# ffreyer/MonteCarlo.jl

Hardware: AMD Instinct MI355X
Metric: DQMC sweeps/sec, 16x16 Hubbard beta=8 dtau=0.1; achieved % fp64 MFMA roofline (higher is better)
Workload: dtype f64

## Files before the change

### montecarlo.jl_amd/csrc/engine.cpp

```cpp
#include <hip/hip_runtime.h>

#include <algorithm>
#include <cmath>
#include <cstdio>
#include <cstdlib>
#include <cstring>
#include <string>
#include <vector>

#include "../../include/dqmc_hip.h"
#include "kernels.h"
#include <rccl/rccl.h>

using namespace dqmc;

struct dqmc_comm {
    ncclComm_t comm = nullptr;
    int nranks = 1, rank = 0, device = 0;
};

static thread_local std::string g_create_error;

struct UTStack;

// ... 374 lines not shown
    if (const char *e = getenv("DQMC_QRB_SITES")) k.qrb_sites = atoi(e) & 7;
    if (const char *e = getenv("DQMC_QR_TAIL")) k.qr_tail = atoi(e) != 0;
    k.qr_sc1 = getenv("DQMC_QR_SC1") != nullptr;
    k.qr_nocoop = getenv("DQMC_QR_NOCOOP") != nullptr;
    if (const char *e = getenv("DQMC_QR_FORCE_TIMEOUT"))
        k.qr_force_timeout = strncmp(e, "step:", 5) == 0 ? 2 + atoi(e + 5) : (strncmp(e, "extra:", 6) == 0 ? 1000 + atoi(e + 6) : 1);
    k.qr_nopanel = getenv("DQMC_QR_NOPANEL") != nullptr;
    k.trsm_simple = getenv("DQMC_TRSM_SIMPLE") != nullptr;
    k.sweep_split = getenv("DQMC_SWEEP_SPLIT") != nullptr;
    k.flush_ncp2 = getenv("DQMC_FLUSH_NCP2") != nullptr;
    k.no_slab = getenv("DQMC_NO_SLAB") != nullptr;
    k.no_kron = getenv("DQMC_NO_KRON") != nullptr;
    k.no_wrap_flush = getenv("DQMC_NO_WRAP_FLUSH") != nullptr;
    k.wrap_two_launch = getenv("DQMC_WRAP_TWO_LAUNCH") != nullptr;
    k.tdm_general = getenv("DQMC_TDM_GENERAL") != nullptr;
}

static int alloc_qr_workspace(dqmc_handle *h)
{
    CHK(dalloc(h, &h->qr_ws.errflag, (size_t)1));
    h->qr_ws.tail = h->sw.qr_tail;
    h->qr_ws.force_sc1 = h->sw.qr_sc1;
    h->qr_ws.no_coop = h->sw.qr_nocoop;
    h->qr_ws.no_panel = h->sw.qr_nopanel;
    h->qr_ws.force_timeout = h->sw.qr_force_timeout;
    if (h->n > 256) return 0;
    hipDeviceProp_t prop;
    HIPCHK(hipGetDeviceProperties(&prop, h->p.device_id));
    const size_t slots = (size_t)((h->units + 7) / 8) * 8 * QR_COOP_SLOTS_PER_UNIT;
    CHK(dalloc(h, &h->qr_ws.mailbox, slots * QR_COOP_SLOT));
// ... 89 lines not shown
    if (udt_is_fused(h, 0) && Tout && Tout != A) return udt_fused(h, A, Uout, Dout, Tout, apply, h->qs[0]);
    CHK(udt_factor(h, A, Dout, Tout, apply, h->qs[0]));
    return udt_formq(h, Uout, h->qs[0], h->qs[0].winv, h->qs[0].ts);
}
static int rdivp_set(dqmc_handle *h, const double *A, const double *T, double *Out, const QrSet &q, double *winv, double *ts)
{
    Timed t(h, DQMC_K_TRSM);
    HIPCHK(launch_trsm_right_upper(h->n, h->units, A, h->nn, T, h->nn, q.pivot, nullptr, 0, Out, h->nn, winv, h->sw, h->cur, ts));
    return 0;
}
static int rdivp(dqmc_handle *h, double *A, const double *T)
{
    return rdivp_set(h, A, T, A, h->qs[0], h->qs[0].winv, h->qs[0].ts);
}

static int calculate_greens_src(dqmc_handle *h, double *out, Udt L, Udt R, double *a2_copy = nullptr)
{
    const int n = h->n;
    QrSet &qa = h->qs[0], &qb = h->qs[0];
    GemmArgs g = gemm_base(h, U_(h, L.t), 0, U_(h, R.t), 1, out);
    g.colscale = vs_arr(R.d, n);
    g.rowscale = vs_arr(L.d, n);
    CHK(run_gemm(h, g));
    if (udt_is_fused(h, 1)) {
        if (L.u == h->Tl) return fail(h, DQMC_ERR_STATE, "calculate_greens: Ul aliases Tl");
        CHK(udt_fused(h, out, h->Tl, h->Dr, qa.W, 0, qa, L.u));
        CHK(rdivp_set(h, R.u, qa.W, h->Ur, qa, qa.winv, qa.ts));
    } else {
        CHK(udt_factor(h, out, h->Dr, nullptr, 0, qa));
        CHK(rdivp_set(h, R.u, out, h->Ur, qa, qa.winv, qa.ts));
        CHK(udt_formq(h, h->Tr, qa, qa.winv, qa.ts));
// ... 4 lines not shown
    CHK(run_gemm(h, g));
    if (a2_copy) CHK(copy_mat(h, a2_copy, h->Tr));
    const double *tlul = h->Tr;
    if (udt_is_fused(h, 2)) {
        CHK(udt_fused(h, h->Tr, h->Ul, h->Dr, qb.W, 0, qb, h->Tl));
        CHK(rdivp_set(h, h->Ur, qb.W, h->Ur, qb, qb.winv, qb.ts));
        tlul = h->Ul;
    } else {
        CHK(udt_factor(h, h->Tr, h->Dr, nullptr, 0, qb));
        CHK(rdivp_set(h, h->Ur, h->Tr, h->Ur, qb, qb.winv, qb.ts));
        CHK(udt_formq(h, h->Ul, qb, qb.winv, qb.ts));
        CHK(run_gemm(h, gemm_base(h, U_(h, h->Tl), 0, U_(h, h->Ul), 0, h->Tr)));
    }
    g = gemm_base(h, U_(h, h->Ur), 0, U_(h, tlul), 1, out);
    g.kscale = vs_inv(h->Dr, n);
    CHK(run_gemm(h, g));
    return 0;
}
static int calculate_greens(dqmc_handle *h, double *out, double *a2_copy = nullptr)
{
    return calculate_greens_src(h, out, Udt{h->Ul, h->Dl, h->Tl}, Udt{h->Ur, h->Dr, h->Tr}, a2_copy);
}

enum { CB_LEFT_B = 0, CB_LEFT_BINV = 1, CB_LEFT_BDAG = 2, CB_RIGHT_B = 3, CB_RIGHT_BINV = 4, CB_RIGHT_ET = 5,
       CB_LEFT_ETINV = 6 };
static int cb_mult(dqmc_handle *h, int which, int slice, const double *X, double *O, const double *qscale)
{
    CbArgs a{};
    a.n = h->n; a.nb = h->nb; a.kmax = h->cb.kmax;
    a.side = (which == CB_RIGHT_B || which == CB_RIGHT_BINV || which == CB_RIGHT_ET) ? 1 : 0;
// ... 271 lines not shown
}

static int reset_slot(dqmc_handle *h, int slot)
{
    const int sp = h->K + 1;
    CHK(set_identity(h, uslot(h, sp)));
    CHK(set_ones(h, dslot(h, sp)));
    CHK(set_identity(h, tslot(h, sp)));
    slot_swap_spare(h, slot);
    return 0;
}
static int prop_check(dqmc_handle *h)
{
    Timed t(h, DQMC_K_MISC);
    HIPCHK(launch_prop_check(h->n, h->nb, h->W, h->greens_temp, h->greens, h->nn, h->stats, h->pc_scratch, h->cur));
    return 0;
}

static int init_stack(dqmc_handle *h)
{
    CHK(set_identity(h, h->Ul)); CHK(set_identity(h, h->Ur));
    CHK(set_identity(h, h->Tl)); CHK(set_identity(h, h->Tr));
    CHK(set_ones(h, h->Dl)); CHK(set_ones(h, h->Dr));
    h->current_slice = 0;
    h->direction = 0;
    return 0;
}
static int build_stack(dqmc_handle *h)
{
    CHK(reset_slot(h, 0));
// ... 15 lines not shown
                discard_pending_flush(h);
                CHK(calculate_greens_src(h, h->greens, slot_ref(h, 0), R));
            } else if (1 < h->current_slice && h->current_slice <= M) {
                const int idx = (h->current_slice - 1) / s;
                const Udt R = slot_ref(h, idx);
                const bool wt = h->p.check_propagation_error != 0, wt_slab = wt && oop_wrap(h);
                CHK(add_slice_sequence_left(h, idx, wt_slab));
                const Udt L = slot_ref(h, idx);
                if (wt && !wt_slab) {
                    CHK(materialize_pending_flush(h));
                    CHK(copy_mat(h, h->greens_temp, h->greens));
                    CHK(wrap_greens(h, &h->greens_temp, h->current_slice - 1, 1));
                }
                if (wt_slab) {
                    std::swap(h->greens, h->greens_alt);
                    CHK(calculate_greens_src(h, h->greens, L, R));
                    CHK(prop_check(h));
                    return 0;
                }
                discard_pending_flush(h);
                CHK(calculate_greens_src(h, h->greens, L, R));
                if (h->p.check_propagation_error) CHK(prop_check(h));
            } else {
                CHK(add_slice_sequence_left(h, h->K));
                h->direction = -1;
                h->current_slice = M + 1;
                CHK(propagate(h));
            }
        } else {
            CHK(wrap_greens(h, &h->greens, h->current_slice, 1));
            h->current_slice += 1;
        }
    } else {
        if ((h->current_slice - 1) % s == 0) {
            h->current_slice -= 1;
            if (h->current_slice == M) {
                const Udt L = slot_ref(h, h->K);
                CHK(reset_slot(h, h->K));
                discard_pending_flush(h);
                CHK(calculate_greens_src(h, h->greens, L, slot_ref(h, h->K)));
                CHK(wrap_greens(h, &h->greens, h->current_slice + 1, -1));
            } else if (0 < h->current_slice && h->current_slice < M) {
                const int idx = h->current_slice / s + 1;
                const Udt L = slot_ref(h, idx - 1);
                CHK(add_slice_sequence_right(h, idx));
                const Udt R = slot_ref(h, idx - 1);
                if (h->p.check_propagation_error) {
                    CHK(materialize_pending_flush(h));
                    std::swap(h->greens_temp, h->greens);
                }
                discard_pending_flush(h);
                CHK(calculate_greens_src(h, h->greens, L, R));
                if (h->p.check_propagation_error) CHK(prop_check(h));
                CHK(wrap_greens(h, &h->greens, h->current_slice + 1, -1));
            } else {
                CHK(add_slice_sequence_right(h, 1));
                h->direction = 1;
                h->current_slice = 0;
                CHK(propagate(h));
            }
        } else {
            CHK(wrap_greens(h, &h->greens, h->current_slice, -1));
            h->current_slice -= 1;
        }
    }
    return 0;
}

// ... 1239 lines not shown
```

### montecarlo.jl_amd/csrc/gemm_f64.hip

```cpp
#include "kernels.h"
#include <hip/hip_ext.h>
#include <cstdlib>

namespace dqmc {

typedef double d4 __attribute__((ext_vector_type(4)));

constexpr int BM = 64, BN = 64, BK = 16;
constexpr int LS = 80;

template <bool KCONTIG, bool FULL>
__device__ __forceinline__ void tile_load(const double *__restrict__ p, int ld, int c0, int cdim,
                                          int k0, int kdim, int tid, double r[4])
{
    if (FULL) {
        const double *q = KCONTIG ? p + (long)ld * (c0 + (tid >> 2)) + k0 + ((tid & 3) << 2)
                                  : p + (long)ld * (k0 + (tid >> 4)) + c0 + ((tid & 15) << 2);
        r[0] = q[0]; r[1] = q[1]; r[2] = q[2]; r[3] = q[3];
        return;
    }
    if (!KCONTIG) {
        const int kk = k0 + (tid >> 4), cc = c0 + ((tid & 15) << 2);
        const double *q = p + (long)ld * kk + cc;
        if (kk < kdim && cc + 3 < cdim) {
// ... 18 lines not shown
__device__ __forceinline__ void tile_store(double (*Xs)[LS], int tid, const double r[4])
{
    if (!KCONTIG) {
        const int k = tid >> 4;
        double *d = &Xs[k][(((tid & 15) << 2) + ((k >> 2) << 2)) & 63];
        d[0] = r[0]; d[1] = r[1]; d[2] = r[2]; d[3] = r[3];
    } else {
        const int c = tid >> 2, k = (tid & 3) << 2;
#pragma unroll
        for (int i = 0; i < 4; ++i) Xs[k + i][(c + k) & 63] = r[i];
    }
}

#define GEMM_LDS_BARRIER() asm volatile("s_waitcnt lgkmcnt(0)\n\ts_barrier" ::: "memory")

template <bool TA, bool TB, bool FULL, int KSM>
__global__ __launch_bounds__(256) void gemm_kernel(GemmArgs g, int tiles_m, int tiles_n)
{
    __shared__ double As[2][BK][LS];
    __shared__ double Bs[2][BK][LS];

    const int bid = blockIdx.x, xcd = bid & 7, seq = bid >> 3;
    const int T = tiles_m * tiles_n;
    const int unit = (seq / T) * 8 + xcd;
    if (unit >= g.n_units) return;
    const int tile = seq % T;
    int m0 = (tile % tiles_m) * BM, n0 = (tile / tiles_m) * BN;
    int kbeg = 0, kend = g.K;
    if (g.tri == 1) {
        if (m0 > n0) return;
// ... 10 lines not shown
    const int tid = threadIdx.x, lane = tid & 63, wave = tid >> 6;
    const int wm = (wave & 1) * 32, wn = (wave >> 1) * 32;
    const int li = lane & 15, lq = lane >> 4;

    d4 acc[2][2];
#pragma unroll
    for (int i = 0; i < 2; ++i)
#pragma unroll
        for (int j = 0; j < 2; ++j) acc[i][j] = (d4){0.0, 0.0, 0.0, 0.0};

    const int nk = (kend - kbeg + BK - 1) / BK;
    double ra[2][4], rb[2][4];
    constexpr int NKS = TA ? 4 : 1;
    double ksd[2][NKS];
    int ksc[2][NKS];
    const int ksmode = KSM >= 0 ? KSM : g.kscale.mode;
    const int kw = unit / g.nb, kblk = unit - kw * g.nb;

    auto load = [&](int kt, double (&qa)[4], double (&qb)[4], double (&qd)[NKS], int (&qc)[NKS]) {
        const int k0 = kbeg + kt * BK;
        tile_load<TA, FULL>(A, g.A.ld, m0, g.M, k0, g.K, tid, qa);
        tile_load<!TB, FULL>(B, g.B.ld, n0, g.N, k0, g.K, tid, qb);
        if (ksmode != 0) {
            const int kb = TA ? k0 + ((tid & 3) << 2) : k0 + (tid >> 4);
#pragma unroll
            for (int i = 0; i < NKS; ++i) {
                const int kk = min(kb + i, g.K - 1);
                if (ksmode == 2) qc[i] = g.kscale.conf[(long)kw * g.kscale.conf_stride + kk];
                else qd[i] = g.kscale.d[(long)unit * g.kscale.stride + kk];
            }
        }
// ... 20 lines not shown
        tile_store<!TB>(Bs[buf], tid, qb);
    };
    auto compute = [&](int cur) {
#pragma unroll
        for (int kk = 0; kk < BK; kk += 4) {
            const int kq = kk + lq, rot = kk;
            const double a0 = As[cur][kq][(wm + li + rot) & 63], a1 = As[cur][kq][(wm + 16 + li + rot) & 63];
            const double b0 = Bs[cur][kq][(wn + li + rot) & 63], b1 = Bs[cur][kq][(wn + 16 + li + rot) & 63];
            acc[0][0] = __builtin_amdgcn_mfma_f64_16x16x4f64(b0, a0, acc[0][0], 0, 0, 0);
            acc[1][0] = __builtin_amdgcn_mfma_f64_16x16x4f64(b0, a1, acc[1][0], 0, 0, 0);
            acc[0][1] = __builtin_amdgcn_mfma_f64_16x16x4f64(b1, a0, acc[0][1], 0, 0, 0);
            acc[1][1] = __builtin_amdgcn_mfma_f64_16x16x4f64(b1, a1, acc[1][1], 0, 0, 0);
        }
    };

    load(0, ra[0], rb[0], ksd[0], ksc[0]);
    store(0, ra[0], rb[0], ksd[0], ksc[0]);
    GEMM_LDS_BARRIER();
    load(min(1, nk - 1), ra[1], rb[1], ksd[1], ksc[1]);
    for (int kt = 0; kt < nk; kt += 2) {
        load(min(kt + 2, nk - 1), ra[0], rb[0], ksd[0], ksc[0]);
        compute(0);
        if (kt + 1 < nk) store(1, ra[1], rb[1], ksd[1], ksc[1]);
        GEMM_LDS_BARRIER();
        if (kt + 1 >= nk) break;
        load(min(kt + 3, nk - 1), ra[1], rb[1], ksd[1], ksc[1]);
        compute(1);
        if (kt + 2 < nk) store(0, ra[0], rb[0], ksd[0], ksc[0]);
        GEMM_LDS_BARRIER();
    }

    const bool plain = g.rowscale.mode == 0 && g.colscale.mode == 0 && g.adddiag.mode == 0 && m0 + BM <= g.M &&
                       n0 + BN <= g.N;
    if (plain) {
        double cold[2][2][4];
        if (g.beta) {
#pragma unroll
            for (int ti = 0; ti < 2; ++ti)
#pragma unroll
                for (int tj = 0; tj < 2; ++tj)
#pragma unroll
                    for (int r = 0; r < 4; ++r)
                        cold[ti][tj][r] = C[(long)g.ldc * (n0 + wn + tj * 16 + lq + 4 * r) + m0 + wm + ti * 16 + li];
        }
#pragma unroll
        for (int ti = 0; ti < 2; ++ti) {
            const int m = m0 + wm + ti * 16 + li;
#pragma unroll
            for (int tj = 0; tj < 2; ++tj) {
#pragma unroll
                for (int r = 0; r < 4; ++r) {
                    const int n = n0 + wn + tj * 16 + lq + 4 * r;
                    double v = acc[ti][tj][r] * g.alpha;
                    if (m == n) v += g.ident;
                    if (g.beta) v += cold[ti][tj][r];
                    C[(long)g.ldc * n + m] = v;
                }
            }
        }
        return;
    }
    if (g.rowscale.mode <= 1 && g.colscale.mode <= 1 && g.adddiag.mode <= 1) {
        const double *csd = g.colscale.mode ? g.colscale.d + (long)unit * g.colscale.stride : nullptr;
        const double *rsd = g.rowscale.mode ? g.rowscale.d + (long)unit * g.rowscale.stride : nullptr;
        const double *add = g.adddiag.mode ? g.adddiag.d + (long)unit * g.adddiag.stride : nullptr;
        double csv[2][4] = {{1.0, 1.0, 1.0, 1.0}, {1.0, 1.0, 1.0, 1.0}}, rsv[2] = {1.0, 1.0}, adv[2] = {0.0, 0.0}, cold[2][2][4];
        const int mc0 = min(m0 + wm + li, g.M - 1), mc1 = min(m0 + wm + 16 + li, g.M - 1);
        if (csd) {
#pragma unroll
            for (int tj = 0; tj < 2; ++tj)
#pragma unroll
                for (int r = 0; r < 4; ++r) csv[tj][r] = csd[min(n0 + wn + tj * 16 + lq + 4 * r, g.N - 1)];
        }
        if (rsd) { rsv[0] = rsd[mc0]; rsv[1] = rsd[mc1]; }
// ... 11 lines not shown
        }
#pragma unroll
        for (int ti = 0; ti < 2; ++ti) {
            const int m = m0 + wm + ti * 16 + li;
#pragma unroll
            for (int tj = 0; tj < 2; ++tj)
#pragma unroll
                for (int r = 0; r < 4; ++r) {
                    const int n = n0 + wn + tj * 16 + lq + 4 * r;
                    double v = acc[ti][tj][r];
                    if (g.row_first) { v *= rsv[ti]; v *= csv[tj][r]; } else { v *= csv[tj][r]; v *= rsv[ti]; }
                    v *= g.alpha;
                    if (m == n) v += g.ident + adv[ti];
                    if (g.beta) v += cold[ti][tj][r];
                    if (m < g.M && n < g.N) C[(long)g.ldc * n + m] = v;
                }
        }
        return;
    }
    double csv[2][4];
#pragma unroll
    for (int tj = 0; tj < 2; ++tj)
#pragma unroll
        for (int r = 0; r < 4; ++r) {
            const int n = n0 + wn + tj * 16 + lq + 4 * r;
            csv[tj][r] = (g.colscale.mode && n < g.N) ? vs_get(g.colscale, unit, g.nb, n) : 1.0;
        }
#pragma unroll
    for (int ti = 0; ti < 2; ++ti) {
        const int m = m0 + wm + ti * 16 + li;
        if (m >= g.M) continue;
        const double rs = g.rowscale.mode ? vs_get(g.rowscale, unit, g.nb, m) : 1.0;
// ... 2 lines not shown
#pragma unroll
            for (int r = 0; r < 4; ++r) {
                const int n = n0 + wn + tj * 16 + lq + 4 * r;
                if (n >= g.N) continue;
                double v = acc[ti][tj][r];
                const double cs = csv[tj][r];
                if (g.row_first) { v *= rs; v *= cs; } else { v *= cs; v *= rs; }
                v *= g.alpha;
                if (m == n) {
                    v += g.ident;
                    if (g.adddiag.mode) v += vs_get(g.adddiag, unit, g.nb, m);
                }
                double *c = C + (long)g.ldc * n + m;
                if (g.beta) v += *c;
                *c = v;
            }
        }
    }
}

hipError_t launch_gemm(const GemmArgs &g, hipStream_t s, hipEvent_t start, hipEvent_t stop)
{
    const int tm = (g.M + BM - 1) / BM, tn = (g.N + BN - 1) / BN;
    const int groups = (g.n_units + 7) / 8;
    dim3 grid(groups * 8 * tm * tn), block(256);
    const bool full = g.M % BM == 0 && g.N % BN == 0 && g.K % BK == 0;
#define GEMM_LAUNCH4(TA, TB, FU, KS) \
    hipExtLaunchKernelGGL((gemm_kernel<TA, TB, FU, KS>), grid, block, 0, s, start, stop, 0, g, tm, tn)
#define GEMM_LAUNCH(TA, TB)                                                        \
    do {                                                                           \
        if (!full) GEMM_LAUNCH4(TA, TB, false, -1);                                \
        else if (g.kscale.mode == 0) GEMM_LAUNCH4(TA, TB, true, 0);                \
        else if (g.kscale.mode == 2) GEMM_LAUNCH4(TA, TB, true, 2);                \
        else if (g.kscale.mode == 1) GEMM_LAUNCH4(TA, TB, true, 1);                \
        else if (g.kscale.mode == 3) GEMM_LAUNCH4(TA, TB, true, 3);                \
        else if (g.kscale.mode == 4) GEMM_LAUNCH4(TA, TB, true, 4);                \
        else if (g.kscale.mode == 5) GEMM_LAUNCH4(TA, TB, true, 5);                \
        else GEMM_LAUNCH4(TA, TB, true, -1);                                       \
    } while (0)
    if (g.transA) {
        if (g.transB) GEMM_LAUNCH(true, true);
        else GEMM_LAUNCH(true, false);
    } else {
        if (g.transB) GEMM_LAUNCH(false, true);
        else GEMM_LAUNCH(false, false);
    }
#undef GEMM_LAUNCH
#undef GEMM_LAUNCH4
    return hipGetLastError();
}

__global__ __launch_bounds__(256) void mfma_peak_kernel(int iters, double *sink)
{
    d4 a0 = {0, 0, 0, 0}, a1 = a0, a2 = a0, a3 = a0;
    double x = 1.0 + threadIdx.x * 1e-9, y = 1.0 - threadIdx.x * 1e-9;
// ... 17 lines not shown
```

### montecarlo.jl_amd/csrc/kernels.h

```cpp
#pragma once
#include <hip/hip_runtime.h>
#include <stdint.h>

namespace dqmc {

struct VecSrc {
    int mode;
    const double *d;
    long stride;
    const int8_t *conf;
    long conf_stride;
    double cpos[2], cneg[2];
};
static inline VecSrc vs_none() { VecSrc v = {}; v.mode = 0; return v; }
static inline VecSrc vs_arr(const double *d, long stride) { VecSrc v = {}; v.mode = 1; v.d = d; v.stride = stride; return v; }
static inline VecSrc vs_inv(const double *d, long stride) { VecSrc v = {}; v.mode = 3; v.d = d; v.stride = stride; return v; }
static inline VecSrc vs_min1(const double *d, long stride) { VecSrc v = {}; v.mode = 4; v.d = d; v.stride = stride; return v; }
static inline VecSrc vs_maxinv(const double *d, long stride) { VecSrc v = {}; v.mode = 5; v.d = d; v.stride = stride; return v; }
#ifdef __HIPCC__
__device__ __forceinline__ double vs_get(const VecSrc &v, int unit, int nb, int i)
{
    if (v.mode == 1) return v.d[(long)unit * v.stride + i];
    if (v.mode == 3) return 1.0 / v.d[(long)unit * v.stride + i];
    if (v.mode == 2) {
// ... 14 lines not shown
};
static inline MatRef mat(const double *p, long su, int ld, long sb = 0) { MatRef m = {p, su, sb, ld}; return m; }

struct GemmArgs {
    int M, N, K;
    int n_units, nb;
    MatRef A, B;
    double *C; long strideC; int ldc;
    int transA, transB;
    VecSrc kscale, colscale, rowscale, adddiag;
    int row_first;
    double alpha;
    double ident;
    int beta;
    int tri;
};
hipError_t launch_gemm(const GemmArgs &g, hipStream_t s, hipEvent_t start = nullptr, hipEvent_t stop = nullptr);
constexpr int SLAB_MAX_STEPS = 10;
struct SlabStep {
    const double *A; long su, sb;
    const int8_t *pre_conf; int pre_sign;
    const int8_t *post_conf; int post_sign;
};
struct SlabArgs {
    int n_units, nb, nsteps;
    SlabStep st[SLAB_MAX_STEPS];
    const double *X0; long x_su, x_sb;
    double *out; long out_su;
    const double *col_d; long col_stride;
    const int8_t *col_conf; int col_sign;
// ... 33 lines not shown
    bool qr_noblocked = false;
    int qrb_sites = 7;
    bool qr_tail = true;
    bool qr_sc1 = false;
    bool qr_nocoop = false;
    int qr_force_timeout = 0;
    bool qr_nopanel = false;
    bool trsm_simple = false;
    bool sweep_split = false;
    bool flush_ncp2 = false;
    bool no_slab = false;
    bool no_kron = false;
    bool no_wrap_flush = false;
    bool wrap_two_launch = false;
    bool tdm_general = false;
};

constexpr int QR_COOP_SLOT = 528;
constexpr int QR_COOP_SLOTS_PER_UNIT = 16;
struct QrCoopWorkspace {
    double *mailbox = nullptr;
    int *errflag = nullptr;
    int *fb = nullptr;
    unsigned long long epoch = 0;
    int max_blocks = 0;
    bool tail = true;
    int force_sc1 = 0;
    int no_coop = 0;
    bool no_panel = false;
    int force_timeout = 0;
// ... 70 lines not shown
        c0 = n0; c1 = n1; c2 = n2; c3 = n3;
        k0 += 0x9E3779B9u;
        k1 += 0xBB67AE85u;
    }
    const unsigned long long hi = c0 >> 5, lo = c1 >> 6;
    return (double)((hi << 26) | lo) * (1.0 / 9007199254740992.0);
}

__device__ __forceinline__ void magstats_push(DevMagStats &s, double value)
{
    const double v = log10(fabs(value));
    s.max = fmax(s.max, v);
    s.min = fmin(s.min, v);
    s.sum += v;
    s.count += 1;
}
#endif
size_t sweep_lu_image_doubles();
constexpr int LU_TILE = 256;
constexpr int LU_OFF_U = 0, LU_OFF_L = 6 * LU_TILE, LU_OFF_PT = 12 * LU_TILE, LU_OFF_Q = 16 * LU_TILE;
constexpr int LU_IMG = 20 * LU_TILE;
constexpr int LU_STRIDE = LU_IMG + 64;
__host__ __device__ constexpr int lu_pair(int K, int J)
{
    return K == 0 ? J - 1 : (K == 1 ? J + 1 : 5);
}
hipError_t launch_sweep_lu(int n, int nb, int n_walkers, const double *G, long strideG, int8_t *conf_slice,
                           long conf_stride, int site0, int nsites, double *img, SweepConsts sc, WalkerRng *rng,
                           DevStats *stats, int check_sign, int *errflag, hipStream_t s,
                           hipEvent_t start = nullptr, hipEvent_t stop = nullptr);
// ... 110 lines not shown
```

### montecarlo.jl_amd/csrc/qr.hip

```cpp
#include "kernels.h"
#include <cstdlib>

namespace dqmc {

__device__ __forceinline__ double wave_sum(double x)
{
#pragma unroll
    for (int off = 32; off > 0; off >>= 1) x += __shfl_xor(x, off, 64);
    return x;
}

constexpr int QR_THREADS = 1024;
constexpr int QR_WAVES = QR_THREADS / 64;

template <int QMAX, int QR_UC>
__global__ __launch_bounds__(QR_THREADS) void qr_pivot_kernel(int n, double *__restrict__ Aall, long strideA,
                                                             double *__restrict__ tauall,
                                                             int *__restrict__ pivall,
                                                             const double *__restrict__ srcall, long strideSrc,
                                                             int *guard, int guard_val)
{
    extern __shared__ __attribute__((aligned(16))) double sm[];
    if (guard && guard[0] != guard_val) return;
    if (srcall) {
// ... 1683 lines not shown
                                                          double *__restrict__ Wall, int nblk)
{
    __shared__ double B[16][17], rdg[16];
    const int J = blockIdx.x, unit = blockIdx.y, j = threadIdx.x, j0 = J << 4;
    const double *__restrict__ T = Tall + (long)unit * sT;
    const double *__restrict__ dmul = dmulall ? dmulall + (long)unit * sV : nullptr;
    double *__restrict__ W = Wall + ((long)unit * nblk + J) * 256;
    const int col = j0 + j;
    {
        const int cc = min(col, n - 1);
        double bv[16], dv;
#pragma unroll
        for (int i = 0; i < 16; ++i) bv[i] = T[min(j0 + i, n - 1) + (long)n * cc];
        dv = dmul ? dmul[cc] : T[cc + (long)n * cc];
        asm volatile("" ::: "memory");
#pragma unroll
        for (int i = 0; i < 16; ++i) B[i][j] = (col < n && j0 + i < n && i < j) ? bv[i] : 0.0;
        rdg[j] = col < n ? (dmul ? dv : 1.0 / dv) : 1.0;
    }
    __syncthreads();
    double wcol[16];
#pragma unroll
    for (int i = 15; i >= 0; --i) {
        double sum = (i == j) ? 1.0 : 0.0;
#pragma unroll
        for (int kk = i + 1; kk < 16; ++kk) sum -= B[i][kk] * ((kk <= j) ? wcol[kk] : 0.0);
        wcol[i] = (i <= j) ? sum * rdg[i] : 0.0;
    }
#pragma unroll
    for (int i = 0; i < 16; ++i) W[i + 16 * j] = wcol[i];
}

__global__ void trsm_gather_kernel(int n, const double *__restrict__ Aall, long sA, const int *__restrict__ pivall,
                                   double *__restrict__ Wall, long sW)
{
    const int unit = blockIdx.y;
    const double *__restrict__ A = Aall + (long)unit * sA;
    double *__restrict__ W = Wall + (long)unit * sW;
    const int *__restrict__ piv = pivall ? pivall + (long)unit * n : nullptr;
    const long nn = (long)n * n;
    for (long idx = blockIdx.x * (long)blockDim.x + threadIdx.x; idx < nn; idx += (long)gridDim.x * blockDim.x) {
        const int r = (int)(idx % n), c = (int)(idx / n);
        W[idx] = A[r + (long)n * (piv ? piv[c] : c)];
    }
}

hipError_t launch_trsm_rl(int nr, int nc, int c0, int ld, int nblk_all, int n_units, const double *A, long sA,
                          const double *T, long sT, const int *pivot, double *Out, long sO, const double *winv,
                          hipStream_t s);

hipError_t launch_trsm_right_upper(int n, int n_units, const double *A, long sA, const double *T, long sT,
                                   const int *pivot, const double *dmul, long sV, double *Out, long sO,
                                   double *winv, const KernelSwitches &sw, hipStream_t s, double *scratch)
{
    const bool no_mfma = sw.trsm_simple;
    if (n <= 256 && winv && !no_mfma) {
        const int nblk = (n + 15) / 16;
        hipLaunchKernelGGL(trsm_diag_inv_kernel, dim3(nblk, n_units), dim3(16), 0, s, n, T, sT, dmul, sV, winv, nblk);
        return launch_trsm_rl(n, n, 0, n, nblk, n_units, A, sA, T, sT, pivot, Out, sO, winv, s);
    }
    if (n > 256 && winv && scratch && sA == sO && !no_mfma) {
        const int nblk = (n + 15) / 16;
        int pw = 256;
        for (int cand = 256; cand >= 128; cand -= 16)
            if (n % cand == 0) { pw = cand; break; }
        hipLaunchKernelGGL(trsm_diag_inv_kernel, dim3(nblk, n_units), dim3(16), 0, s, n, T, sT, dmul, sV, winv, nblk);
        int bx = (int)(((long)n * n + 255) / 256);
        if (bx > 128) bx = 128;
        hipLaunchKernelGGL(trsm_gather_kernel, dim3(bx, n_units), dim3(256), 0, s, n, A, sA, pivot, scratch, sO);
        for (int c0 = 0; c0 < n; c0 += pw) {
            const int nc = n - c0 < pw ? n - c0 : pw;
            if (c0 > 0) {
                GemmArgs g{};
                g.M = n; g.N = nc; g.K = c0;
// ... 38 lines not shown
```

### montecarlo.jl_amd/csrc/sweep.hip

```cpp
#include "kernels.h"

namespace dqmc {

__global__ void set_identity_kernel(int n, double *A, long stride)
{
    double *a = A + (long)blockIdx.y * stride;
    const long nn = (long)n * n;
    for (long idx = blockIdx.x * (long)blockDim.x + threadIdx.x; idx < nn; idx += (long)gridDim.x * blockDim.x) {
        const int r = (int)(idx % n), c = (int)(idx / n);
        a[idx] = r == c ? 1.0 : 0.0;
    }
}
hipError_t launch_set_identity(int n, int count, double *A, long stride, hipStream_t s)
{
    const long nn = (long)n * n;
    int bx = (int)((nn + 255) / 256);
    if (bx > 64) bx = 64;
    hipLaunchKernelGGL(set_identity_kernel, dim3(bx, count), dim3(256), 0, s, n, A, stride);
    return hipGetLastError();
}
__global__ void set_diag_kernel(int n, int nb, double *A, long stride, VecSrc d)
{
    const int unit = blockIdx.y;
    double *a = A + (long)unit * stride;
// ... 106 lines not shown
        const double *a = A + (long)w * tot, *b = B + (long)w * tot;
        for (long i = (long)part * blockDim.x + threadIdx.x; i < tot; i += (long)PC_SPLIT * blockDim.x) {
            const double e0 = fabs(a[i] - b[i]);
            bad |= (e0 != e0);
            d = fmax(d, e0);
        }
    } else {
        const double2 *a = reinterpret_cast<const double2 *>(A + (long)w * tot), *b = reinterpret_cast<const double2 *>(B + (long)w * tot);
        for (long i = (long)part * blockDim.x + threadIdx.x; i < tot / 2; i += (long)PC_SPLIT * blockDim.x) {
            const double2 x = a[i], y = b[i];
            const double e0 = fabs(x.x - y.x), e1 = fabs(x.y - y.y);
            bad |= (e0 != e0) | (e1 != e1);
            d = fmax(d, fmax(e0, e1));
        }
    }
    if (bad) d = __longlong_as_double(0x7ff8000000000000ll);
#pragma unroll
    for (int off = 32; off > 0; off >>= 1) {
        const double o = __shfl_xor(d, off, 64);
        d = (d != d || o != o) ? __longlong_as_double(0x7ff8000000000000ll) : fmax(d, o);
    }
    if ((threadIdx.x & 63) == 0) red[threadIdx.x >> 6] = d;
    __syncthreads();
    if (threadIdx.x == 0) {
        for (int i = 1; i < (int)(blockDim.x >> 6); ++i) d = (d != d || red[i] != red[i]) ? __longlong_as_double(0x7ff8000000000000ll) : fmax(d, red[i]);
        atomicMax(&scratch[2 * w], (unsigned long long)__double_as_longlong(d));
        __threadfence();
        if (atomicAdd(&scratch[2 * w + 1], 1ull) == PC_SPLIT - 1) {
            __threadfence();
            const double m = __longlong_as_double((long long)atomicExch(&scratch[2 * w], 0ull));
            scratch[2 * w + 1] = 0ull;
            if (m > 1e-7) magstats_push(stats[w].propagation_error, m);
        }
    }
}
hipError_t launch_prop_check(int n, int nb, int n_walkers, const double *A, const double *B, long stride_unit,
                             DevStats *stats, unsigned long long *scratch, hipStream_t s)
{
    hipLaunchKernelGGL(prop_check_kernel, dim3(n_walkers * PC_SPLIT), dim3(1024), 0, s, n, nb, A, B, stride_unit, stats,
                       scratch);
    return hipGetLastError();
}

__global__ void accumulate_kernel(int n, int nb, int n_walkers, const double *__restrict__ G, long stride_unit,
                                  double *__restrict__ acc)
{
    const long per = (long)nb * n * n;
    for (long e = blockIdx.x * (long)blockDim.x + threadIdx.x; e < per; e += (long)gridDim.x * blockDim.x) {
// ... 278 lines not shown
```

### montecarlo.jl_amd/csrc/trsm_rl.hip

```cpp
#include "kernels.h"
#include <type_traits>

namespace dqmc {

typedef double d4_t __attribute__((ext_vector_type(4)));

#ifdef TR_STAMPS
__device__ long long *tr_stamp_ptr = nullptr;
#define TR_STAMP(idx)                                                                                        \
    do {                                                                                                     \
        if (blockIdx.x == 0 && (threadIdx.x & 63) == 0 && tr_stamp_ptr)                                      \
            tr_stamp_ptr[(threadIdx.x >> 6) * 64 + (idx)] = (long long)__builtin_amdgcn_s_memtime();         \
    } while (0)
#else
#define TR_STAMP(idx) do { } while (0)
#endif
constexpr int TR_TS = 18;
template <bool FULLB>
__global__ __launch_bounds__(256) void trsm_rl_kernel(int nr, int n, int c0, int ld, int nblk_all,
                                                     const double *__restrict__ Aall, long sA,
                                                     const double *__restrict__ Tall, long sT,
                                                     const int *__restrict__ pivall, double *__restrict__ Oall, long sO,
                                                     int slabs, const double *__restrict__ Wall, int n_units)
{
    extern __shared__ __attribute__((aligned(16))) double trl_sm[];
    double (*Tl)[256 * TR_TS] = reinterpret_cast<double (*)[256 * TR_TS]>(trl_sm);
    double (*Xi)[2][4 * 64] = reinterpret_cast<double (*)[2][4 * 64]>(trl_sm + 3 * 256 * TR_TS);
    double (*Wl)[4 * 64] = reinterpret_cast<double (*)[4 * 64]>(trl_sm + 3 * 256 * TR_TS + 2 * 2 * 256);
    const int bid = blockIdx.x, xcd = bid & 7, seq = bid >> 3;
    const int unit = (seq / slabs) * 8 + xcd, row0 = (seq % slabs) * 32;
    if (unit >= n_units) return;
    const double *__restrict__ A = Aall + (long)unit * sA;
    const double *__restrict__ T = Tall + (long)unit * sT + (long)ld * c0 + c0;
    const int *__restrict__ piv = pivall ? pivall + (long)unit * ld : nullptr;
    double *__restrict__ O = Oall + (long)unit * sO;
    const int tid = threadIdx.x, lane = tid & 63, w = tid >> 6, g = lane >> 4, ci = lane & 15;
    const int rt = w & 1, par = w >> 1;
    const int nblk = FULLB ? 16 : (n + 15) >> 4;
    const double *__restrict__ Wu = Wall + ((long)unit * nblk_all + (c0 >> 4)) * 256;
    const int row = row0 + 16 * rt + ci;
    const int rowc = min(row, nr - 1);

    TR_STAMP(0);
    d4_t x[8];
    int pjv[8][4];
#pragma unroll
    for (int t = 0; t < 8; ++t)
#pragma unroll
        for (int r = 0; r < 4; ++r) {
            const int cc = min(16 * (2 * t + par) + 4 * r + g, n - 1);
            pjv[t][r] = piv ? piv[c0 + cc] : c0 + cc;
        }
#pragma unroll
    for (int t = 0; t < 8; ++t)
#pragma unroll
        for (int r = 0; r < 4; ++r) x[t][r] = A[(unsigned)(rowc + ld * pjv[t][r])];
    asm volatile("" ::: "memory");
#pragma unroll
// ... 38 lines not shown
        constexpr int J = decltype(Jc)::value, t_own = J >> 1;
        d4_t o = {0.0, 0.0, 0.0, 0.0};
#pragma unroll
        for (int q = 0; q < 4; ++q) o = __builtin_amdgcn_mfma_f64_16x16x4f64(Wl[J][q * 64 + lane], x[t_own][q], o, 0, 0, 0);
#pragma unroll
        for (int r = 0; r < 4; ++r) {
            Xi[J & 1][rt][r * 64 + lane] = o[r];
            const int col = 16 * J + 4 * r + g;
            if (FULLB || (row < nr && col < n)) O[(unsigned)(row + ld * (c0 + col))] = o[r];
        }
    };
#define TRL_IC(K) std::integral_constant<int, (K)>{}
    request(TRL_IC(0));
    request(TRL_IC(1));
    request(TRL_IC(2));
    {
        const int q = tid >> 6, l = tid & 63, src = (4 * q + (l >> 4)) + 16 * (l & 15);
        double wv[16];
#pragma unroll
        for (int J = 0; J < 16; ++J) wv[J] = Wu[(unsigned)((FULLB ? J : min(J, nblk - 1)) * 256 + src)];
#pragma unroll
        for (int J = 0; J < 16; ++J) Wl[J][tid] = wv[J];
    }
#ifdef TR_STAMPS
    TR_STAMP(42);
    asm volatile("s_waitcnt vmcnt(0)" ::: "memory");
    TR_STAMP(43);
#endif
    deposit(TRL_IC(0));
    TR_STAMP(44);
    __syncthreads();
// ... 36 lines not shown
        if (par == 0) body(TRL_IC(0));
        else body(TRL_IC(1));
        deposit(TRL_IC(J + 2));
        request(TRL_IC(J + 4));
        TR_STAMP(2 + 2 * J);
        asm volatile("s_waitcnt lgkmcnt(0)\n\ts_barrier" ::: "memory");
        TR_STAMP(3 + 2 * J);
    };
#define TRL_STEP(K) step(std::integral_constant<int, K>{})
    TRL_STEP(0); TRL_STEP(1); TRL_STEP(2); TRL_STEP(3); TRL_STEP(4); TRL_STEP(5); TRL_STEP(6); TRL_STEP(7);
    TRL_STEP(8); TRL_STEP(9); TRL_STEP(10); TRL_STEP(11); TRL_STEP(12); TRL_STEP(13); TRL_STEP(14); TRL_STEP(15);
#undef TRL_STEP
#undef TRL_IC
    TR_STAMP(34);
}
#ifdef TR_STAMPS
extern "C" int dqmc_debug_tr_stamps(void *devptr)
{
    return (int)hipMemcpyToSymbol(HIP_SYMBOL(tr_stamp_ptr), &devptr, sizeof(void *));
}
#endif

hipError_t launch_trsm_rl(int nr, int nc, int c0, int ld, int nblk_all, int n_units, const double *A, long sA,
                          const double *T, long sT, const int *pivot, double *Out, long sO, const double *winv,
                          hipStream_t s)
{
    if (nc > 256 || nc < 1) return hipErrorInvalidValue;
    const size_t lds_r = (3 * 256 * TR_TS + 2 * 2 * 256 + 16 * 256) * sizeof(double);
    int dev = 0;
    (void)hipGetDevice(&dev);
    static unsigned attr_mask = 0;
    if (!(attr_mask & (1u << dev))) {
        (void)hipFuncSetAttribute((const void *)trsm_rl_kernel<true>, hipFuncAttributeMaxDynamicSharedMemorySize, (int)lds_r);
        (void)hipFuncSetAttribute((const void *)trsm_rl_kernel<false>, hipFuncAttributeMaxDynamicSharedMemorySize, (int)lds_r);
        attr_mask |= 1u << dev;
    }
    const int slabs = (nr + 31) / 32;
    const int groups = (n_units + 7) / 8;
    if (nc == 256 && nr % 32 == 0)
        hipLaunchKernelGGL(trsm_rl_kernel<true>, dim3(groups * 8 * slabs), dim3(256), lds_r, s, nr, nc, c0, ld, nblk_all, A, sA, T,
                           sT, pivot, Out, sO, slabs, winv, n_units);
    else
        hipLaunchKernelGGL(trsm_rl_kernel<false>, dim3(groups * 8 * slabs), dim3(256), lds_r, s, nr, nc, c0, ld, nblk_all, A, sA,
                           T, sT, pivot, Out, sO, slabs, winv, n_units);
    return hipGetLastError();
}

}
```

Baseline: 810.5.

## Fold propagation check into final greens GEMM and diag-inverse into TRSM

Two fusions. The propagation-error check, which was a separate kernel comparing the new greens with greens_temp, now runs inside the epilogue of the last GEMM of calculate_greens, with a per-block reduction and an atomic arrival counter. Separately, the 16x16 diagonal-block inverse that a standalone trsm_diag_inv_kernel used to compute is now computed inside the TRSM kernel's prologue. Both remove a kernel launch and a global round trip, at the cost of extra registers and work in the GEMM and TRSM kernels, which may affect occupancy.

Result: no change. 815.4 (median of 6 runs) (+0.6%).

```diff
diff --git a/montecarlo.jl_amd/csrc/engine.cpp b/montecarlo.jl_amd/csrc/engine.cpp
--- a/montecarlo.jl_amd/csrc/engine.cpp
+++ b/montecarlo.jl_amd/csrc/engine.cpp
@@ -412,6 +412,7 @@
     k.no_wrap_flush = getenv("DQMC_NO_WRAP_FLUSH") != nullptr;
     k.wrap_two_launch = getenv("DQMC_WRAP_TWO_LAUNCH") != nullptr;
     k.tdm_general = getenv("DQMC_TDM_GENERAL") != nullptr;
+    k.no_fold = getenv("DQMC_NO_FOLD") != nullptr;
 }
 
 static int alloc_qr_workspace(dqmc_handle *h)
@@ -531,7 +532,8 @@
     return rdivp_set(h, A, T, A, h->qs[0], h->qs[0].winv, h->qs[0].ts);
 }
 
-static int calculate_greens_src(dqmc_handle *h, double *out, Udt L, Udt R, double *a2_copy = nullptr)
+static int calculate_greens_src(dqmc_handle *h, double *out, Udt L, Udt R, double *a2_copy = nullptr,
+                                const double *check_against = nullptr)
 {
     const int n = h->n;
     QrSet &qa = h->qs[0], &qb = h->qs[0];
@@ -566,6 +568,11 @@
     }
     g = gemm_base(h, U_(h, h->Ur), 0, U_(h, tlul), 1, out);
     g.kscale = vs_inv(h->Dr, n);
+    if (check_against) {
+        g.cmp = check_against;
+        g.cmp_stats = h->stats;
+        g.cmp_scratch = h->pc_scratch;
+    }
     CHK(run_gemm(h, g));
     return 0;
 }
@@ -867,6 +874,13 @@
 {
     Timed t(h, DQMC_K_MISC);
     HIPCHK(launch_prop_check(h->n, h->nb, h->W, h->greens_temp, h->greens, h->nn, h->stats, h->pc_scratch, h->cur));
+    return 0;
+}
+static int calculate_greens_checked(dqmc_handle *h, Udt L, Udt R)
+{
+    const bool check = h->p.check_propagation_error != 0, fold = check && !h->sw.no_fold;
+    CHK(calculate_greens_src(h, h->greens, L, R, nullptr, fold ? h->greens_temp : nullptr));
+    if (check && !fold) CHK(prop_check(h));
     return 0;
 }
 
@@ -912,13 +926,11 @@
                 }
                 if (wt_slab) {
                     std::swap(h->greens, h->greens_alt);
-                    CHK(calculate_greens_src(h, h->greens, L, R));
-                    CHK(prop_check(h));
+                    CHK(calculate_greens_checked(h, L, R));
                     return 0;
                 }
                 discard_pending_flush(h);
-                CHK(calculate_greens_src(h, h->greens, L, R));
-                if (h->p.check_propagation_error) CHK(prop_check(h));
+                CHK(calculate_greens_checked(h, L, R));
             } else {
                 CHK(add_slice_sequence_left(h, h->K));
                 h->direction = -1;
@@ -948,8 +960,7 @@
                     std::swap(h->greens_temp, h->greens);
                 }
                 discard_pending_flush(h);
-                CHK(calculate_greens_src(h, h->greens, L, R));
-                if (h->p.check_propagation_error) CHK(prop_check(h));
+                CHK(calculate_greens_checked(h, L, R));
                 CHK(wrap_greens(h, &h->greens, h->current_slice + 1, -1));
             } else {
                 CHK(add_slice_sequence_right(h, 1));
diff --git a/montecarlo.jl_amd/csrc/gemm_f64.hip b/montecarlo.jl_amd/csrc/gemm_f64.hip
--- a/montecarlo.jl_amd/csrc/gemm_f64.hip
+++ b/montecarlo.jl_amd/csrc/gemm_f64.hip
@@ -56,6 +56,7 @@
 
 #define GEMM_LDS_BARRIER() asm volatile("s_waitcnt lgkmcnt(0)\n\ts_barrier" ::: "memory")
 
+constexpr int GEMM_KSM_CHECK3 = 6, GEMM_KSM_CHECK_ANY = -2;
 template <bool TA, bool TB, bool FULL, int KSM>
 __global__ __launch_bounds__(256) void gemm_kernel(GemmArgs g, int tiles_m, int tiles_n)
 {
@@ -96,7 +97,8 @@
     constexpr int NKS = TA ? 4 : 1;
     double ksd[2][NKS];
     int ksc[2][NKS];
-    const int ksmode = KSM >= 0 ? KSM : g.kscale.mode;
+    constexpr bool CHECK = KSM == GEMM_KSM_CHECK3 || KSM == GEMM_KSM_CHECK_ANY;
+    const int ksmode = KSM == GEMM_KSM_CHECK3 ? 3 : (KSM >= 0 ? KSM : g.kscale.mode);
     const int kw = unit / g.nb, kblk = unit - kw * g.nb;
 
     auto load = [&](int kt, double (&qa)[4], double (&qb)[4], double (&qd)[NKS], int (&qc)[NKS]) {
@@ -147,6 +149,21 @@
         }
     };
 
+    const double *__restrict__ R = CHECK ? g.cmp + (long)unit * g.strideC : nullptr;
+    double cref[2][2][4], pc_d = 0.0;
+    bool pc_bad = false;
+    if constexpr (CHECK) {
+#pragma unroll
+        for (int ti = 0; ti < 2; ++ti)
+#pragma unroll
+            for (int tj = 0; tj < 2; ++tj)
+#pragma unroll
+                for (int r = 0; r < 4; ++r) {
+                    const int m = FULL ? m0 + wm + ti * 16 + li : min(m0 + wm + ti * 16 + li, g.M - 1);
+                    const int n = FULL ? n0 + wn + tj * 16 + lq + 4 * r : min(n0 + wn + tj * 16 + lq + 4 * r, g.N - 1);
+                    cref[ti][tj][r] = R[(long)g.ldc * n + m];
+                }
+    }
     load(0, ra[0], rb[0], ksd[0], ksc[0]);
     store(0, ra[0], rb[0], ksd[0], ksc[0]);
     GEMM_LDS_BARRIER();
@@ -163,6 +180,26 @@
         GEMM_LDS_BARRIER();
     }
 
+    auto pc_take = [&](double v, double ref, bool inside) {
+        if constexpr (CHECK) {
+            asm("" : "+v"(v));
+            const double e = fabs(ref - v);
+            pc_bad |= inside && (e != e);
+            pc_d = fmax(pc_d, inside ? e : 0.0);
+        }
+    };
+    auto pc_finish = [&]() {
+        if constexpr (CHECK) {
+            double d = prop_check_wave_max(pc_bad ? prop_check_nan() : pc_d);
+            double *red = &As[0][0][0];
+            if (lane == 0) red[wave] = d;
+            __syncthreads();
+            if (tid == 0) {
+                for (int i = 1; i < 4; ++i) d = prop_check_max(d, red[i]);
+                prop_check_arrive(g.cmp_stats, g.cmp_scratch, kw, d, (unsigned long long)T * g.nb);
+            }
+        }
+    };
     const bool plain = g.rowscale.mode == 0 && g.colscale.mode == 0 && g.adddiag.mode == 0 && m0 + BM <= g.M &&
                        n0 + BN <= g.N;
     if (plain) {
@@ -188,9 +225,11 @@
                     if (m == n) v += g.ident;
                     if (g.beta) v += cold[ti][tj][r];
                     C[(long)g.ldc * n + m] = v;
+                    pc_take(v, cref[ti][tj][r], true);
                 }
             }
         }
+        pc_finish();
         return;
     }
     if (g.rowscale.mode <= 1 && g.colscale.mode <= 1 && g.adddiag.mode <= 1) {
@@ -232,8 +271,10 @@
                     if (m == n) v += g.ident + adv[ti];
                     if (g.beta) v += cold[ti][tj][r];
                     if (m < g.M && n < g.N) C[(long)g.ldc * n + m] = v;
+                    pc_take(v, cref[ti][tj][r], m < g.M && n < g.N);
                 }
         }
+        pc_finish();
         return;
     }
     double csv[2][4];
@@ -266,9 +307,11 @@
                 double *c = C + (long)g.ldc * n + m;
                 if (g.beta) v += *c;
                 *c = v;
-            }
-        }
-    }
+                pc_take(v, cref[ti][tj][r], true);
+            }
+        }
+    }
+    pc_finish();
 }
 
 hipError_t launch_gemm(const GemmArgs &g, hipStream_t s, hipEvent_t start, hipEvent_t stop)
@@ -290,7 +333,12 @@
         else if (g.kscale.mode == 5) GEMM_LAUNCH4(TA, TB, true, 5);                \
         else GEMM_LAUNCH4(TA, TB, true, -1);                                       \
     } while (0)
-    if (g.transA) {
+    if (g.cmp) {
+        if (g.transA || !g.transB || g.tri || !g.cmp_stats || !g.cmp_scratch) return hipErrorInvalidValue;
+        if (full && g.kscale.mode == 3) GEMM_LAUNCH4(false, true, true, GEMM_KSM_CHECK3);
+        else if (full) GEMM_LAUNCH4(false, true, true, GEMM_KSM_CHECK_ANY);
+        else GEMM_LAUNCH4(false, true, false, GEMM_KSM_CHECK_ANY);
+    } else if (g.transA) {
         if (g.transB) GEMM_LAUNCH(true, true);
         else GEMM_LAUNCH(true, false);
     } else {
diff --git a/montecarlo.jl_amd/csrc/kernels.h b/montecarlo.jl_amd/csrc/kernels.h
--- a/montecarlo.jl_amd/csrc/kernels.h
+++ b/montecarlo.jl_amd/csrc/kernels.h
@@ -52,6 +52,9 @@
     double ident;
     int beta;
     int tri;
+    const double *cmp;
+    struct DevStats *cmp_stats;
+    unsigned long long *cmp_scratch;
 };
 hipError_t launch_gemm(const GemmArgs &g, hipStream_t s, hipEvent_t start = nullptr, hipEvent_t stop = nullptr);
 constexpr int SLAB_MAX_STEPS = 10;
@@ -115,6 +118,7 @@
     bool no_wrap_flush = false;
     bool wrap_two_launch = false;
     bool tdm_general = false;
+    bool no_fold = false;
 };
 
 constexpr int QR_COOP_SLOT = 528;
@@ -215,6 +219,43 @@
     s.min = fmin(s.min, v);
     s.sum += v;
     s.count += 1;
+}
+__device__ __forceinline__ double prop_check_nan() { return __longlong_as_double(0x7ff8000000000000ll); }
+__device__ __forceinline__ double prop_check_max(double a, double b) { return (a != a || b != b) ? prop_check_nan() : fmax(a, b); }
+__device__ __forceinline__ double prop_check_wave_max(double d)
+{
+#pragma unroll
+    for (int off = 32; off > 0; off >>= 1) d = prop_check_max(d, __shfl_xor(d, off, 64));
+    return d;
+}
+__device__ __forceinline__ void prop_check_arrive(DevStats *stats, unsigned long long *scratch, int w, double d,
+                                                  unsigned long long target)
+{
+    const unsigned long long before = atomicMax(&scratch[2 * w], (unsigned long long)__double_as_longlong(d));
+    asm volatile("" ::"v"(before) : "memory");
+    if (atomicAdd(&scratch[2 * w + 1], 1ull) == target - 1) {
+        const double m = __longlong_as_double((long long)atomicExch(&scratch[2 * w], 0ull));
+        scratch[2 * w + 1] = 0ull;
+        if (m > 1e-7) magstats_push(stats[w].propagation_error, m);
+    }
+}
+__device__ __forceinline__ void trsm_diag_inv_deposit(double (*B)[17], double *rdg, int j0, int j, int n, const double bv[16],
+                                                      double dv, bool dv_is_reciprocal)
+{
+    const int col = j0 + j;
+#pragma unroll
+    for (int i = 0; i < 16; ++i) B[i][j] = (col < n && j0 + i < n && i < j) ? bv[i] : 0.0;
+    rdg[j] = col < n ? (dv_is_reciprocal ? dv : 1.0 / dv) : 1.0;
+}
+__device__ __forceinline__ void trsm_diag_inv_column(const double (*B)[17], const double *rdg, int j, double wcol[16])
+{
+#pragma unroll
+    for (int i = 15; i >= 0; --i) {
+        double sum = (i == j) ? 1.0 : 0.0;
+#pragma unroll
+        for (int kk = i + 1; kk < 16; ++kk) sum -= B[i][kk] * ((kk <= j) ? wcol[kk] : 0.0);
+        wcol[i] = (i <= j) ? sum * rdg[i] : 0.0;
+    }
 }
 #endif
 size_t sweep_lu_image_doubles();
diff --git a/montecarlo.jl_amd/csrc/qr.hip b/montecarlo.jl_amd/csrc/qr.hip
--- a/montecarlo.jl_amd/csrc/qr.hip
+++ b/montecarlo.jl_amd/csrc/qr.hip
@@ -1721,19 +1721,11 @@
         for (int i = 0; i < 16; ++i) bv[i] = T[min(j0 + i, n - 1) + (long)n * cc];
         dv = dmul ? dmul[cc] : T[cc + (long)n * cc];
         asm volatile("" ::: "memory");
-#pragma unroll
-        for (int i = 0; i < 16; ++i) B[i][j] = (col < n && j0 + i < n && i < j) ? bv[i] : 0.0;
-        rdg[j] = col < n ? (dmul ? dv : 1.0 / dv) : 1.0;
+        trsm_diag_inv_deposit(B, rdg, j0, j, n, bv, dv, dmul != nullptr);
     }
     __syncthreads();
     double wcol[16];
-#pragma unroll
-    for (int i = 15; i >= 0; --i) {
-        double sum = (i == j) ? 1.0 : 0.0;
-#pragma unroll
-        for (int kk = i + 1; kk < 16; ++kk) sum -= B[i][kk] * ((kk <= j) ? wcol[kk] : 0.0);
-        wcol[i] = (i <= j) ? sum * rdg[i] : 0.0;
-    }
+    trsm_diag_inv_column(B, rdg, j, wcol);
 #pragma unroll
     for (int i = 0; i < 16; ++i) W[i + 16 * j] = wcol[i];
 }
@@ -1763,8 +1755,10 @@
     const bool no_mfma = sw.trsm_simple;
     if (n <= 256 && winv && !no_mfma) {
         const int nblk = (n + 15) / 16;
-        hipLaunchKernelGGL(trsm_diag_inv_kernel, dim3(nblk, n_units), dim3(16), 0, s, n, T, sT, dmul, sV, winv, nblk);
-        return launch_trsm_rl(n, n, 0, n, nblk, n_units, A, sA, T, sT, pivot, Out, sO, winv, s);
+        const bool fold = !dmul && !sw.no_fold;
+        if (!fold)
+            hipLaunchKernelGGL(trsm_diag_inv_kernel, dim3(nblk, n_units), dim3(16), 0, s, n, T, sT, dmul, sV, winv, nblk);
+        return launch_trsm_rl(n, n, 0, n, nblk, n_units, A, sA, T, sT, pivot, Out, sO, fold ? nullptr : winv, s);
     }
     if (n > 256 && winv && scratch && sA == sO && !no_mfma) {
         const int nblk = (n + 15) / 16;
diff --git a/montecarlo.jl_amd/csrc/sweep.hip b/montecarlo.jl_amd/csrc/sweep.hip
--- a/montecarlo.jl_amd/csrc/sweep.hip
+++ b/montecarlo.jl_amd/csrc/sweep.hip
@@ -144,24 +144,13 @@
             d = fmax(d, fmax(e0, e1));
         }
     }
-    if (bad) d = __longlong_as_double(0x7ff8000000000000ll);
-#pragma unroll
-    for (int off = 32; off > 0; off >>= 1) {
-        const double o = __shfl_xor(d, off, 64);
-        d = (d != d || o != o) ? __longlong_as_double(0x7ff8000000000000ll) : fmax(d, o);
-    }
+    if (bad) d = prop_check_nan();
+    d = prop_check_wave_max(d);
     if ((threadIdx.x & 63) == 0) red[threadIdx.x >> 6] = d;
     __syncthreads();
     if (threadIdx.x == 0) {
-        for (int i = 1; i < (int)(blockDim.x >> 6); ++i) d = (d != d || red[i] != red[i]) ? __longlong_as_double(0x7ff8000000000000ll) : fmax(d, red[i]);
-        atomicMax(&scratch[2 * w], (unsigned long long)__double_as_longlong(d));
-        __threadfence();
-        if (atomicAdd(&scratch[2 * w + 1], 1ull) == PC_SPLIT - 1) {
-            __threadfence();
-            const double m = __longlong_as_double((long long)atomicExch(&scratch[2 * w], 0ull));
-            scratch[2 * w + 1] = 0ull;
-            if (m > 1e-7) magstats_push(stats[w].propagation_error, m);
-        }
+        for (int i = 1; i < (int)(blockDim.x >> 6); ++i) d = prop_check_max(d, red[i]);
+        prop_check_arrive(stats, scratch, w, d, PC_SPLIT);
     }
 }
 hipError_t launch_prop_check(int n, int nb, int n_walkers, const double *A, const double *B, long stride_unit,
diff --git a/montecarlo.jl_amd/csrc/trsm_rl.hip b/montecarlo.jl_amd/csrc/trsm_rl.hip
--- a/montecarlo.jl_amd/csrc/trsm_rl.hip
+++ b/montecarlo.jl_amd/csrc/trsm_rl.hip
@@ -16,12 +16,12 @@
 #define TR_STAMP(idx) do { } while (0)
 #endif
 constexpr int TR_TS = 18;
-template <bool FULLB>
-__global__ __launch_bounds__(256) void trsm_rl_kernel(int nr, int n, int c0, int ld, int nblk_all,
-                                                     const double *__restrict__ Aall, long sA,
-                                                     const double *__restrict__ Tall, long sT,
-                                                     const int *__restrict__ pivall, double *__restrict__ Oall, long sO,
-                                                     int slabs, const double *__restrict__ Wall, int n_units)
+template <bool FULLB, bool INV>
+__device__ __forceinline__ void trsm_rl_body(int nr, int n, int c0, int ld, int nblk_all,
+                                             const double *__restrict__ Aall, long sA,
+                                             const double *__restrict__ Tall, long sT,
+                                             const int *__restrict__ pivall, double *__restrict__ Oall, long sO,
+                                             int slabs, const double *__restrict__ Wall, int n_units)
 {
     extern __shared__ __attribute__((aligned(16))) double trl_sm[];
     double (*Tl)[256 * TR_TS] = reinterpret_cast<double (*)[256 * TR_TS]>(trl_sm);
@@ -37,11 +37,17 @@
     const int tid = threadIdx.x, lane = tid & 63, w = tid >> 6, g = lane >> 4, ci = lane & 15;
     const int rt = w & 1, par = w >> 1;
     const int nblk = FULLB ? 16 : (n + 15) >> 4;
-    const double *__restrict__ Wu = Wall + ((long)unit * nblk_all + (c0 >> 4)) * 256;
     const int row = row0 + 16 * rt + ci;
     const int rowc = min(row, nr - 1);
 
     TR_STAMP(0);
+    double dbv[16], ddv = 1.0;
+    if constexpr (INV) {
+        const int j0 = 16 * (4 * w + g), cc = min(j0 + ci, n - 1);
+#pragma unroll
+        for (int i = 0; i < 16; ++i) dbv[i] = T[(unsigned)(ld * cc + min(j0 + i, n - 1))];
+        ddv = T[(unsigned)(ld * cc + cc)];
+    }
     d4_t x[8];
     int pjv[8][4];
 #pragma unroll
@@ -110,7 +116,21 @@
     request(TRL_IC(0));
     request(TRL_IC(1));
     request(TRL_IC(2));
-    {
+    if constexpr (INV) {
+        double (*Bi)[16][17] = reinterpret_cast<double (*)[16][17]>(Tl[2]);
+        double *rdg = Tl[2] + 16 * 16 * 17;
+        static_assert(16 * 16 * 17 + 256 == 256 * TR_TS, "block staging must fit the third panel buffer");
+        const int Jb = 4 * w + g;
+        trsm_diag_inv_deposit(Bi[Jb], rdg + 16 * Jb, 16 * Jb, ci, n, dbv, ddv, false);
+        __builtin_amdgcn_fence(__ATOMIC_RELEASE, "wavefront");
+        __builtin_amdgcn_wave_barrier();
+        __builtin_amdgcn_fence(__ATOMIC_ACQUIRE, "wavefront");
+        double wcol[16];
+        trsm_diag_inv_column(Bi[Jb], rdg + 16 * Jb, ci, wcol);
+#pragma unroll
+        for (int i = 0; i < 16; ++i) Wl[Jb][(i >> 2) * 64 + (i & 3) * 16 + ci] = wcol[i];
+    } else {
+        const double *__restrict__ Wu = Wall + ((long)unit * nblk_all + (c0 >> 4)) * 256;
         const int q = tid >> 6, l = tid & 63, src = (4 * q + (l >> 4)) + 16 * (l & 15);
         double wv[16];
 #pragma unroll
@@ -177,6 +197,17 @@
 #undef TRL_IC
     TR_STAMP(34);
 }
+#define TRL_PARAMS                                                                                                        \
+    int nr, int n, int c0, int ld, int nblk_all, const double *__restrict__ Aall, long sA, const double *__restrict__ Tall, \
+        long sT, const int *__restrict__ pivall, double *__restrict__ Oall, long sO, int slabs,                           \
+        const double *__restrict__ Wall, int n_units
+#define TRL_ARGS nr, n, c0, ld, nblk_all, Aall, sA, Tall, sT, pivall, Oall, sO, slabs, Wall, n_units
+template <bool FULLB>
+__global__ __launch_bounds__(256) void trsm_rl_kernel(TRL_PARAMS) { trsm_rl_body<FULLB, false>(TRL_ARGS); }
+template <bool FULLB>
+__global__ __launch_bounds__(256) void trsm_rl_inv_kernel(TRL_PARAMS) { trsm_rl_body<FULLB, true>(TRL_ARGS); }
+#undef TRL_PARAMS
+#undef TRL_ARGS
 #ifdef TR_STAMPS
 extern "C" int dqmc_debug_tr_stamps(void *devptr)
 {
@@ -189,6 +220,8 @@
                           hipStream_t s)
 {
     if (nc > 256 || nc < 1) return hipErrorInvalidValue;
+    const bool inv = winv == nullptr;
+    if (inv && (c0 != 0 || nr != nc || ld != nc)) return hipErrorInvalidValue;
     const size_t lds_r = (3 * 256 * TR_TS + 2 * 2 * 256 + 16 * 256) * sizeof(double);
     int dev = 0;
     (void)hipGetDevice(&dev);
@@ -196,16 +229,23 @@
     if (!(attr_mask & (1u << dev))) {
         (void)hipFuncSetAttribute((const void *)trsm_rl_kernel<true>, hipFuncAttributeMaxDynamicSharedMemorySize, (int)lds_r);
         (void)hipFuncSetAttribute((const void *)trsm_rl_kernel<false>, hipFuncAttributeMaxDynamicSharedMemorySize, (int)lds_r);
+        (void)hipFuncSetAttribute((const void *)trsm_rl_inv_kernel<true>, hipFuncAttributeMaxDynamicSharedMemorySize, (int)lds_r);
+        (void)hipFuncSetAttribute((const void *)trsm_rl_inv_kernel<false>, hipFuncAttributeMaxDynamicSharedMemorySize, (int)lds_r);
         attr_mask |= 1u << dev;
     }
     const int slabs = (nr + 31) / 32;
     const int groups = (n_units + 7) / 8;
-    if (nc == 256 && nr % 32 == 0)
-        hipLaunchKernelGGL(trsm_rl_kernel<true>, dim3(groups * 8 * slabs), dim3(256), lds_r, s, nr, nc, c0, ld, nblk_all, A, sA, T,
-                           sT, pivot, Out, sO, slabs, winv, n_units);
-    else
-        hipLaunchKernelGGL(trsm_rl_kernel<false>, dim3(groups * 8 * slabs), dim3(256), lds_r, s, nr, nc, c0, ld, nblk_all, A, sA,
-                           T, sT, pivot, Out, sO, slabs, winv, n_units);
+#define TRL_LAUNCH(KERNEL)                                                                                                 \
+    hipLaunchKernelGGL((KERNEL), dim3(groups * 8 * slabs), dim3(256), lds_r, s, nr, nc, c0, ld, nblk_all, A, sA, T, \
+                       sT, pivot, Out, sO, slabs, winv, n_units)
+    if (nc == 256 && nr % 32 == 0) {
+        if (inv) TRL_LAUNCH(trsm_rl_inv_kernel<true>);
+        else TRL_LAUNCH(trsm_rl_kernel<true>);
+    } else {
+        if (inv) TRL_LAUNCH(trsm_rl_inv_kernel<false>);
+        else TRL_LAUNCH(trsm_rl_kernel<false>);
+    }
+#undef TRL_LAUNCH
     return hipGetLastError();
 }
 
```
